# efirdc/Segmentation-Pipeline

Hardware: AMD Instinct MI355X
Metric: 3D patches/sec (128³, 4ch) train+infer at 1/2/4/8 MI355X; Dice vs CPU ref (higher is better)
Workload: dtype f32 (tensors, results and accumulation; the products of the 3x3x3 convolutions with >= 8 input channels run as six bf16 MFMAs on an EXACT three-way bf16 split of both f32 operands -- error vs f64 equal to the f32 MFMA kernels', profiles/r04_f32x3_accuracy.txt; the same step on v_mfma_f32_32x32x2_f32

## Files before the change

### segmentation-pipeline_amd/csrc/conv3d_f32x3.hip

```cpp
#include "conv3d_common.hpp"

namespace m355 {

typedef __bf16 bf16x8 __attribute__((ext_vector_type(8)));
typedef unsigned u32x4 __attribute__((ext_vector_type(4)));

constexpr int X3_PAIRS = 14;
constexpr int X3_QUADS = 7;
__host__ __device__ constexpr int x3_pair_tap(int pair, int half) {
  return pair < 9 ? pair * 3 + half : (pair < 12 ? (pair - 9) * 9 + half * 3 + 2 : (pair == 12 ? half * 9 + 8 : (half ? -1 : 26)));
}

__device__ __forceinline__ void x3_split(float v, unsigned& hi, unsigned& mid, unsigned& lo) {
  const unsigned u = __float_as_uint(v);
  hi = u & 0xffff0000u;
  const float r1 = (u & 0x7f800000u) == 0x7f800000u ? 0.f : v - __uint_as_float(hi);
  mid = __float_as_uint(r1) & 0xffff0000u;
  lo = __float_as_uint(r1 - __uint_as_float(mid));
}
__device__ __forceinline__ unsigned x3_pack(unsigned a, unsigned b) { return __builtin_amdgcn_perm(b, a, 0x07060302u); }

__device__ __forceinline__ void pack_w3_x3_item(const float* __restrict__ w, u32x4* __restrict__ wq, int64_t i, int Cout_w,
                                                int Cin_w, int kin, int mout, int nchunks, int transpose) {
  const int lane = (int)(i & 63);
// ... 987 lines not shown
  const dim3 grid((unsigned)(p.ctiles * p.otiles * p.nsplit));
#define M355_X3_BWW(TXV)                                                                                              \
  hipLaunchKernelGGL((conv3_bww_x3_kernel<TXV>), grid, dim3(512), 0, st, x, dy, slab, N, Cin, Cout, D, H, W, p.ty_tiles, \
                     p.tx_tiles, p.nsplit, p.ctiles, p.otiles, xbs, ybs);
  if (p.tx == 32) { M355_X3_BWW(32) } else if (p.tx == 16) { M355_X3_BWW(16) } else { M355_X3_BWW(8) }
#undef M355_X3_BWW
  return M355_OK;
}

template <int NVT>
__global__ __launch_bounds__(256) void convt_k2s2_fwd_x3_kernel(
    const float* __restrict__ x, const float* __restrict__ w, const float* __restrict__ bias, float* __restrict__ y, int Cin,
    int Cout, int D, int H, int W, int64_t xbs, int64_t ybs, int mt_per_wg) {
  extern __shared__ __attribute__((aligned(16))) unsigned char xs3_raw[];
  u32x4* xs3 = reinterpret_cast<u32x4*>(xs3_raw);
  constexpr int NG = NVT / 32, P = 256 / NVT;
  const int tid = threadIdx.x, lane = tid & 63;
  const int wave = __builtin_amdgcn_readfirstlane(tid >> 6);
  const int half = lane >> 5, l32 = lane & 31;
  const int S = D * H * W;
  const int v0 = blockIdx.x * NVT;
  const int n = blockIdx.z;
  const float* xn = x + (int64_t)n * xbs;
  float* yn = y + (int64_t)n * ybs;
  const int CB = (Cin + 15) / 16 * 2;
  const int OH = 2 * H, OW = 2 * W;
  const int64_t OS = (int64_t)S * 8;
  {
    const int sv = tid % NVT, part = tid / NVT;
    const bool vin = v0 + sv < S;
    const float* xp = xn + (vin ? v0 + sv : 0);
    for (int cb = part; cb < CB; cb += P) {
      float v[8];
#pragma unroll
      for (int j = 0; j < 8; ++j) {
        const int c = cb * 8 + j;
        const bool ok = vin && c < Cin;
        const float t = xp[ok ? (int64_t)c * S : 0];
        v[j] = ok ? t : 0.f;
      }
      unsigned h[8], m[8], l[8];
#pragma unroll
      for (int j = 0; j < 8; ++j) x3_split(v[j], h[j], m[j], l[j]);
      xs3[(0 * CB + cb) * NVT + sv] = (u32x4){x3_pack(h[0], h[1]), x3_pack(h[2], h[3]), x3_pack(h[4], h[5]), x3_pack(h[6], h[7])};
      xs3[(1 * CB + cb) * NVT + sv] = (u32x4){x3_pack(m[0], m[1]), x3_pack(m[2], m[3]), x3_pack(m[4], m[5]), x3_pack(m[6], m[7])};
      xs3[(2 * CB + cb) * NVT + sv] = (u32x4){x3_pack(l[0], l[1]), x3_pack(l[2], l[3]), x3_pack(l[4], l[5]), x3_pack(l[6], l[7])};
    }
  }
  __syncthreads();
  const int mtiles = (Cout + 3) / 4;
  const int mt_begin = blockIdx.y * mt_per_wg, mt_end = min(mtiles, mt_begin + mt_per_wg);
  const int wrow = Cout * 8;
  int64_t obase[NG];
#pragma unroll
  for (int g = 0; g < NG; ++g) {
    const int v = min(v0 + g * 32 + l32, S - 1);
    const int ix = v % W, iy = (v / W) % H, iz = v / (W * H);
    obase[g] = ((int64_t)(2 * iz + half) * OH + 2 * iy) * OW + 2 * ix;
  }
  float a_nxt[8];
  auto wload = [&](int mt, int k0) __attribute__((always_inline)) {
    const int col = min(mt * 32 + l32, Cout * 8 - 1);
#pragma unroll
    for (int j = 0; j < 8; ++j) a_nxt[j] = w[min(k0 + 8 * half + j, Cin - 1) * wrow + col];
  };
  bf16x8 ah, am, al;
  auto wsplit = [&](int mt, int k0) __attribute__((always_inline)) {
    const bool ook = mt * 4 + (l32 >> 3) < Cout;
    unsigned h[8], m[8], l[8];
#pragma unroll
    for (int j = 0; j < 8; ++j) x3_split((ook && k0 + 8 * half + j < Cin) ? a_nxt[j] : 0.f, h[j], m[j], l[j]);
    ah = __builtin_bit_cast(bf16x8, (u32x4){x3_pack(h[0], h[1]), x3_pack(h[2], h[3]), x3_pack(h[4], h[5]), x3_pack(h[6], h[7])});
    am = __builtin_bit_cast(bf16x8, (u32x4){x3_pack(m[0], m[1]), x3_pack(m[2], m[3]), x3_pack(m[4], m[5]), x3_pack(m[6], m[7])});
    al = __builtin_bit_cast(bf16x8, (u32x4){x3_pack(l[0], l[1]), x3_pack(l[2], l[3]), x3_pack(l[4], l[5]), x3_pack(l[6], l[7])});
  };
  const int nchunks = CB / 2;
  int mt = mt_begin + wave;
  if (mt < mt_end) {
    wload(mt, 0);
    wsplit(mt, 0);
  }
  while (mt < mt_end) {
    const int o0 = mt * 4;
    f32x16 acc[NG];
#pragma unroll
    for (int g = 0; g < NG; ++g)
#pragma unroll
      for (int r = 0; r < 16; ++r) acc[g][r] = 0.f;
    for (int ch = 0; ch < nchunks; ++ch) {
      const bool last = ch + 1 >= nchunks;
      const int nmt = last ? mt + 4 : mt, nk0 = last ? 0 : (ch + 1) * 16;
      if (nmt < mt_end) wload(nmt, nk0);
      const u32x4* bp = xs3 + (2 * ch + half) * NVT + l32;
      bf16x8 bh[NG], bm[NG], bl[NG];
#pragma unroll
      for (int g = 0; g < NG; ++g) bh[g] = __builtin_bit_cast(bf16x8, bp[g * 32]);
#pragma unroll
      for (int g = 0; g < NG; ++g) bm[g] = __builtin_bit_cast(bf16x8, bp[CB * NVT + g * 32]);
#pragma unroll
      for (int g = 0; g < NG; ++g) bl[g] = __builtin_bit_cast(bf16x8, bp[2 * CB * NVT + g * 32]);
#pragma unroll
      for (int g = 0; g < NG; ++g) acc[g] = __builtin_amdgcn_mfma_f32_32x32x16_bf16(al, bh[g], acc[g], 0, 0, 0);
#pragma unroll
      for (int g = 0; g < NG; ++g) acc[g] = __builtin_amdgcn_mfma_f32_32x32x16_bf16(am, bh[g], acc[g], 0, 0, 0);
#pragma unroll
      for (int g = 0; g < NG; ++g) acc[g] = __builtin_amdgcn_mfma_f32_32x32x16_bf16(ah, bh[g], acc[g], 0, 0, 0);
#pragma unroll
      for (int g = 0; g < NG; ++g) acc[g] = __builtin_amdgcn_mfma_f32_32x32x16_bf16(am, bm[g], acc[g], 0, 0, 0);
#pragma unroll
      for (int g = 0; g < NG; ++g) acc[g] = __builtin_amdgcn_mfma_f32_32x32x16_bf16(ah, bm[g], acc[g], 0, 0, 0);
#pragma unroll
      for (int g = 0; g < NG; ++g) acc[g] = __builtin_amdgcn_mfma_f32_32x32x16_bf16(ah, bl[g], acc[g], 0, 0, 0);
      wsplit(nmt, nk0);
    }
#pragma unroll
    for (int q = 0; q < 4; ++q) {
      const int o = o0 + q;
      if (o >= Cout) continue;
      const float bv = bias ? bias[o] : 0.f;
      float* yo = yn + (int64_t)o * OS;
#pragma unroll
      for (int g = 0; g < NG; ++g) {
        if (v0 + g * 32 + l32 >= S) continue;
#pragma unroll
        for (int b = 0; b < 2; ++b)
          *reinterpret_cast<float2*>(yo + obase[g] + (int64_t)b * OW) =
              make_float2(acc[g][q * 4 + b * 2] + bv, acc[g][q * 4 + b * 2 + 1] + bv);
      }
    }
    mt += 4;
  }
}

int convt_fwd_x3_nvt(int Cin) {
  const int64_t cin2 = round_up(Cin, 16);
  for (int nvt : {128, 64, 32})
    if (cin2 * nvt * 6 <= 65536) return nvt;
  return 0;
}

void launch_convt_fwd_x3(int nvt, dim3 grid, const float* x, const float* w, const float* bias, float* y, int Cin, int Cout,
                         int D, int H, int W, int64_t xbs, int64_t ybs, int mt_per_wg, hipStream_t st) {
  const size_t lds = (size_t)round_up(Cin, 16) * nvt * 6;
#define M355_CONVT_X3(NVT) \
  hipLaunchKernelGGL(convt_k2s2_fwd_x3_kernel<NVT>, grid, dim3(256), lds, st, x, w, bias, y, Cin, Cout, D, H, W, xbs, ybs, mt_per_wg)
  switch (nvt) {
    case 128: M355_CONVT_X3(128); break;
    case 64: M355_CONVT_X3(64); break;
    default: M355_CONVT_X3(32); break;
  }
#undef M355_CONVT_X3
}

}
```

### segmentation-pipeline_amd/csrc/convt.hip

```cpp
#include "h16.hpp"

namespace m355 {

typedef float f32x16 __attribute__((ext_vector_type(16)));

int convt_fwd_x3_nvt(int Cin);
void launch_convt_fwd_x3(int nvt, dim3 grid, const float* x, const float* w, const float* bias, float* y, int Cin, int Cout,
                         int D, int H, int W, int64_t xbs, int64_t ybs, int mt_per_wg, hipStream_t st);


template <int NVT>
__global__ __launch_bounds__(256) void convt_k2s2_fwd_mfma_kernel(
    const float* __restrict__ x, const float* __restrict__ w, const float* __restrict__ bias,
    float* __restrict__ y, int Cin, int Cout, int D, int H, int W, int64_t xbs, int64_t ybs, int mt_per_wg) {
  extern __shared__ float xs[];
  constexpr int NG = NVT / 32, P = 256 / NVT;
  const int tid = threadIdx.x, lane = tid & 63;
  const int wave = __builtin_amdgcn_readfirstlane(tid >> 6);
  const int half = lane >> 5, l32 = lane & 31;
  const int S = D * H * W;
  const int v0 = blockIdx.x * NVT;
  const int n = blockIdx.z;
  const float* xn = x + (int64_t)n * xbs;
  float* yn = y + (int64_t)n * ybs;
  constexpr int KC = 8;
  const int Cin2 = (Cin + 2 * KC - 1) / (2 * KC) * (2 * KC);
  const int OH = 2 * H, OW = 2 * W;
  const int64_t OS = (int64_t)S * 8;
  {
    const int sv = tid % NVT, part = tid / NVT;
    const bool vin = v0 + sv < S;
    const float* xp = xn + (vin ? v0 + sv : 0);
#pragma unroll 16
    for (int c = part; c < Cin2; c += P) {
      const bool ok = vin && c < Cin;
      const float val = xp[ok ? (int64_t)c * S : 0];
      xs[c * NVT + sv] = ok ? val : 0.f;
    }
  }
  __syncthreads();
  const int mtiles = (Cout + 3) / 4;
  const int mt_begin = blockIdx.y * mt_per_wg, mt_end = min(mtiles, mt_begin + mt_per_wg);
  const int wrow = Cout * 8;
  int64_t obase[NG];
#pragma unroll
  for (int g = 0; g < NG; ++g) {
    const int v = min(v0 + g * 32 + l32, S - 1);
    const int ix = v % W, iy = (v / W) % H, iz = v / (W * H);
    obase[g] = ((int64_t)(2 * iz + half) * OH + 2 * iy) * OW + 2 * ix;
  }
  float a_cur[KC], a_nxt[KC];
  auto wload = [&](float* a, int mt, int k0) {
    const int col = min(mt * 32 + l32, Cout * 8 - 1);
#pragma unroll
    for (int j = 0; j < KC; ++j) a[j] = w[min(k0 + 2 * j + half, Cin - 1) * wrow + col];
  };
  auto wmask = [&](float* dst, const float* src, int mt, int k0) {
    const bool ook = mt * 4 + (l32 >> 3) < Cout;
#pragma unroll
    for (int j = 0; j < KC; ++j) dst[j] = (ook && k0 + 2 * j + half < Cin) ? src[j] : 0.f;
  };
  const float* xb = xs + half * NVT + l32;
  int mt = mt_begin + wave;
  if (mt < mt_end) {
    wload(a_nxt, mt, 0);
    wmask(a_cur, a_nxt, mt, 0);
  }
  while (mt < mt_end) {
    const int o0 = mt * 4;
    f32x16 acc[NG];
#pragma unroll
    for (int g = 0; g < NG; ++g)
#pragma unroll
      for (int r = 0; r < 16; ++r) acc[g][r] = 0.f;
    for (int k0 = 0; k0 < Cin2; k0 += 2 * KC) {
      const bool last = k0 + 2 * KC >= Cin2;
      const int nmt = last ? mt + 4 : mt, nk0 = last ? 0 : k0 + 2 * KC;
      if (nmt < mt_end) wload(a_nxt, nmt, nk0);
      float bq[2][NG];
#pragma unroll
      for (int g = 0; g < NG; ++g) bq[0][g] = xb[k0 * NVT + g * 32];
#pragma unroll
      for (int j = 0; j < KC; ++j) {
        if (j + 1 < KC) {
#pragma unroll
          for (int g = 0; g < NG; ++g) bq[(j + 1) & 1][g] = xb[(k0 + 2 * j + 2) * NVT + g * 32];
        }
        __builtin_amdgcn_sched_barrier(0);
#pragma unroll
        for (int g = 0; g < NG; ++g)
          acc[g] = __builtin_amdgcn_mfma_f32_32x32x2f32(a_cur[j], bq[j & 1][g], acc[g], 0, 0, 0);
        __builtin_amdgcn_sched_barrier(0);
      }
      wmask(a_cur, a_nxt, nmt, nk0);
    }
#pragma unroll
    for (int q = 0; q < 4; ++q) {
      const int o = o0 + q;
      if (o >= Cout) continue;
      const float bv = bias ? bias[o] : 0.f;
      float* yo = yn + (int64_t)o * OS;
#pragma unroll
      for (int g = 0; g < NG; ++g) {
        if (v0 + g * 32 + l32 >= S) continue;
#pragma unroll
        for (int b = 0; b < 2; ++b)
          *reinterpret_cast<float2*>(yo + obase[g] + (int64_t)b * OW) =
              make_float2(acc[g][q * 4 + b * 2] + bv, acc[g][q * 4 + b * 2 + 1] + bv);
      }
    }
    mt += 4;
  }
}

template <int NVT, typename HT>
__global__ __launch_bounds__(256) void convt_k2s2_fwd_c8_kernel(
    const HT* __restrict__ x16, const float* __restrict__ w, const float* __restrict__ bias, HT* __restrict__ y16,
    int Cin, int Cout, int D, int H, int W, int64_t xbs16, int64_t ybs16, int mp_per_wg) {
  using hx8 = typename H16<HT>::x8;
  extern __shared__ float xs[];
  constexpr int NG = NVT / 32, P = 256 / NVT;
  const int tid = threadIdx.x, lane = tid & 63;
  const int wave = __builtin_amdgcn_readfirstlane(tid >> 6);
  const int half = lane >> 5, l32 = lane & 31;
  const int S = D * H * W;
  const int v0 = blockIdx.x * NVT;
  const int n = blockIdx.z;
  constexpr int KC = 8;
  const int Cin2 = (Cin + 2 * KC - 1) / (2 * KC) * (2 * KC);
  const int CBin = (Cin + 7) / 8;
  const int OH = 2 * H, OW = 2 * W;
  const int64_t OS = (int64_t)S * 8;
  {
    const int sv = tid % NVT, part = tid / NVT;
    const bool vin = v0 + sv < S;
    const hx8* xp = reinterpret_cast<const hx8*>(x16 + (int64_t)n * xbs16) + (vin ? v0 + sv : 0);
    for (int cb = part; cb < Cin2 / 8; cb += P) {
      const bool ok = vin && cb < CBin;
      const hx8 v = xp[ok ? (int64_t)cb * S : 0];
#pragma unroll
      for (int j = 0; j < 8; ++j) xs[(cb * 8 + j) * NVT + sv] = (ok && cb * 8 + j < Cin) ? (float)v[j] : 0.f;
    }
  }
  __syncthreads();
  const int mtiles = (Cout + 3) / 4, mpairs = (mtiles + 1) / 2;
  const int mp_begin = blockIdx.y * mp_per_wg, mp_end = min(mpairs, mp_begin + mp_per_wg);
  const int wrow = Cout * 8;
  int64_t obase[NG];
#pragma unroll
  for (int g = 0; g < NG; ++g) {
    const int v = min(v0 + g * 32 + l32, S - 1);
    const int ix = v % W, iy = (v / W) % H, iz = v / (W * H);
    obase[g] = ((int64_t)(2 * iz + half) * OH + 2 * iy) * OW + 2 * ix;
  }
  float a_cur[2][KC], a_nxt[2][KC];
  auto wload = [&](int mp, int k0) {
#pragma unroll
    for (int t = 0; t < 2; ++t) {
      const int col = min((2 * mp + t) * 32 + l32, Cout * 8 - 1);
#pragma unroll
      for (int j = 0; j < KC; ++j) a_nxt[t][j] = w[min(k0 + 2 * j + half, Cin - 1) * wrow + col];
// ... 748 lines not shown
  }
}

__global__ void convt_direct_bwd_data_kernel(const float* __restrict__ dy,
                                             const float* __restrict__ w, float* __restrict__ dx,
                                             int N, int Cin, int Cout, int D, int H, int W, int OD,
                                             int OH, int OW, int k, int stride, int pad,
                                             int64_t xbs, int64_t ybs) {
  const int64_t S = (int64_t)D * H * W;
  const int64_t OS = (int64_t)OD * OH * OW;
  const int64_t total = (int64_t)N * Cin * S;
  const int k3 = k * k * k;
  for (int64_t i = blockIdx.x * (int64_t)blockDim.x + threadIdx.x; i < total;
       i += (int64_t)gridDim.x * blockDim.x) {
    const int ix = (int)(i % W);
    int64_t r = i / W;
    const int iy = (int)(r % H);
    r /= H;
    const int iz = (int)(r % D);
    r /= D;
    const int c = (int)(r % Cin);
    const int n = (int)(r / Cin);
    float acc = 0.f;
    for (int o = 0; o < Cout; ++o) {
      const float* dyo = dy + (int64_t)n * ybs + (int64_t)o * OS;
      const float* wc = w + ((int64_t)c * Cout + o) * k3;
      for (int dz = 0; dz < k; ++dz) {
        const int oz = iz * stride + dz - pad;
        if (oz < 0 || oz >= OD) continue;
        for (int dyy = 0; dyy < k; ++dyy) {
          const int oy = iy * stride + dyy - pad;
          if (oy < 0 || oy >= OH) continue;
          for (int dxx = 0; dxx < k; ++dxx) {
            const int ox = ix * stride + dxx - pad;
            if (ox < 0 || ox >= OW) continue;
            acc = fmaf(dyo[((int64_t)oz * OH + oy) * OW + ox], wc[(dz * k + dyy) * k + dxx], acc);
          }
        }
      }
    }
    dx[(int64_t)n * xbs + (int64_t)c * S + ((int64_t)iz * H + iy) * W + ix] = acc;
  }
}

__global__ __launch_bounds__(256) void convt_direct_bwd_weight_kernel(
    const float* __restrict__ x, const float* __restrict__ dy, float* __restrict__ dw, int N, int Cin,
    int Cout, int D, int H, int W, int OD, int OH, int OW, int k, int stride, int pad, int64_t xbs,
    int64_t ybs) {
  __shared__ double scratch[4];
  const int k3 = k * k * k;
  int b = blockIdx.x;
  const int tap = b % k3;
  b /= k3;
  const int o = b % Cout;
  const int c = b / Cout;
  const int dz = tap / (k * k), dyy = (tap / k) % k, dxx = tap % k;
  const int64_t S = (int64_t)D * H * W;
  const int64_t OS = (int64_t)OD * OH * OW;
  double acc = 0.0;
  for (int n = 0; n < N; ++n) {
    const float* xc = x + (int64_t)n * xbs + (int64_t)c * S;
    const float* dyo = dy + (int64_t)n * ybs + (int64_t)o * OS;
    float part = 0.f;
    int cnt = 0;
    for (int64_t s = threadIdx.x; s < S; s += 256) {
      const int ix = (int)(s % W);
      const int iy = (int)((s / W) % H);
      const int iz = (int)(s / ((int64_t)W * H));
      const int oz = iz * stride + dz - pad, oy = iy * stride + dyy - pad,
                ox = ix * stride + dxx - pad;
      if (oz >= 0 && oz < OD && oy >= 0 && oy < OH && ox >= 0 && ox < OW)
        part = fmaf(xc[s], dyo[((int64_t)oz * OH + oy) * OW + ox], part);
      if (++cnt == 64) { acc += part; part = 0.f; cnt = 0; }
    }
    acc += part;
  }
  const double tot = block_sum<double, 256>(acc, scratch);
  if (threadIdx.x == 0) dw[((int64_t)c * Cout + o) * k3 + tap] = (float)tot;
}

static bool is_k2s2(const m355_conv3d_desc* d) {
  return d->k == 2 && d->stride == 2 && d->pad == 0 && d->out_pad == 0;
}
static int convt_out(int in, const m355_conv3d_desc* d) {
  return (in - 1) * d->stride - 2 * d->pad + d->k + d->out_pad;
}
static int convt_bww_mt(const m355_conv3d_desc* d) { return d->Cin > 64 ? 4 : 2; }
static int convt_nsplit(const m355_conv3d_desc* d) {
  const int64_t tiles = ceil_div(d->Cin, 32 * convt_bww_mt(d)) * ceil_div(d->Cout, 16);
  const int64_t nsteps = ceil_div((int64_t)d->N * d->D * d->H * d->W, 64);
  int64_t ns = std::max<int64_t>(1, 2 * num_cus() / tiles);
  ns = std::min<int64_t>(ns, nsteps);
  return (int)ns;
}
static bool convt_fits_i32(const m355_conv3d_desc* d) {
  return (int64_t)d->D * d->H * d->W * 8 * std::max(d->Cin, d->Cout) < (1ll << 31);
}

static int validate_convt(const m355_conv3d_desc* d, const char* who) {
  M355_REQUIRE(d != nullptr, M355_EINVALID_ARG, "%s: null descriptor", who);
  M355_REQUIRE(d->N > 0 && d->Cin > 0 && d->Cout > 0 && d->D > 0 && d->H > 0 && d->W > 0,
               M355_EINVALID_ARG, "%s: non-positive dimension", who);
  M355_REQUIRE(d->k >= 1 && d->k <= 7 && d->stride >= 1 && d->pad >= 0 && d->out_pad >= 0 &&
                   d->out_pad < d->stride,
               M355_EINVALID_ARG, "%s: bad k/stride/pad/out_pad", who);
  M355_REQUIRE(d->N <= 65535 && d->Cin <= 65535 && d->Cout <= 65535, M355_EUNSUPPORTED,
               "%s: N/Cin/Cout > 65535", who);
  return M355_OK;
}

}

using namespace m355;

int launch_dbias(const float* dy, float* dbias, int N, int Cout, int64_t S, int64_t ybs, void* ws,
                 hipStream_t st);
static size_t convt_slab_bytes(const m355_conv3d_desc* d) {
  return is_k2s2(d) ? (size_t)round_up((int64_t)convt_nsplit(d) * d->Cin * d->Cout * 8 * 4, 256) : 0;
}
static size_t convt_dbias_bytes(const m355_conv3d_desc* d) {
  const int64_t OS = (int64_t)convt_out(d->D, d) * convt_out(d->H, d) * convt_out(d->W, d);
  const int64_t generic = (int64_t)d->Cout * ceil_div(OS, DBIAS_CHUNK) * 8;
  const int64_t fused = is_k2s2(d) ? (int64_t)convt_nsplit(d) * d->Cout * 8 : 0;
  return (size_t)round_up(std::max(generic, fused), 256);
}

static int convt_fwd_nvt(const m355_conv3d_desc* d) {
  const int64_t cin2 = round_up(d->Cin, 16);
  for (int nvt : {128, 64, 32})
    if (cin2 * nvt * 4 <= 65536) return nvt;
  return 0;
}

struct ConvtBwdPlan {
  int mt, nvt, ksplit, o_per_split;
  size_t slab_bytes;
};
static ConvtBwdPlan plan_convt_bwd(const m355_conv3d_desc* d) {
  ConvtBwdPlan p{};
  const int64_t S = (int64_t)d->D * d->H * d->W;
  p.mt = d->Cin > 64 ? 4 : 2;
  const int64_t cblocks = ceil_div(d->Cin, 32 * p.mt);
  p.nvt = 256;
  while (p.nvt > 64 && ceil_div(S, p.nvt) * cblocks * d->N < 512) p.nvt >>= 1;
  const int64_t wgs = ceil_div(S, p.nvt) * cblocks * d->N;
  int64_t ks = 1;
  if (wgs < 256) ks = std::min<int64_t>(std::min<int64_t>(8, ceil_div(512, wgs)), std::max(1, d->Cout / 16));
  p.o_per_split = (int)round_up(ceil_div(d->Cout, ks), 4);
  p.ksplit = (int)ceil_div(d->Cout, p.o_per_split);
  p.slab_bytes = p.ksplit > 1 ? (size_t)round_up((int64_t)p.ksplit * d->N * d->Cin * S * 4, 256) : 0;
  return p;
}

extern "C" size_t m355_conv_transpose3d_workspace(const m355_conv3d_desc* d) {
  if (!d) return 0;
  const size_t bwd = is_k2s2(d) ? plan_convt_bwd(d).slab_bytes : 0;
  return std::max(convt_slab_bytes(d) + convt_dbias_bytes(d), bwd);
}

extern "C" int m355_conv_transpose3d_fwd(const m355_conv3d_desc* d, const float* x, const float* w,
                                         const float* bias, float* y, void* workspace,
                                         size_t workspace_bytes, void* stream) {
  if (int rc = validate_convt(d, "conv_transpose3d_fwd")) return rc;
  M355_REQUIRE(x && w && y, M355_EINVALID_ARG, "conv_transpose3d_fwd: null pointer");
  (void)workspace; (void)workspace_bytes;
  hipStream_t st = (hipStream_t)stream;
  const int OD = convt_out(d->D, d), OH = convt_out(d->H, d), OW = convt_out(d->W, d);
  M355_REQUIRE(OD > 0 && OH > 0 && OW > 0, M355_EINVALID_ARG, "conv_transpose3d_fwd: empty output");
  const int64_t xbs = dense_or(d->x_batch_stride, (int64_t)d->Cin * d->D * d->H * d->W);
  const int64_t ybs = dense_or(d->y_batch_stride, (int64_t)d->Cout * OD * OH * OW);
  const bool x3 = d->compute == M355_COMPUTE_F32X3 && tuning().f32x3 && tuning().f32x3_convt && convt_fwd_x3_nvt(d->Cin) != 0;
  const int nvt = x3 ? convt_fwd_x3_nvt(d->Cin) : convt_fwd_nvt(d);
  if (is_k2s2(d) && nvt && (ybs % 2 == 0) && ((uintptr_t)y & 7) == 0 && convt_fits_i32(d)) {
    const int64_t S = (int64_t)d->D * d->H * d->W;
    const int64_t vox_tiles = ceil_div(S, nvt) * d->N;
    const int mtiles = (int)ceil_div(d->Cout, 4);
    const int64_t groups = std::max<int64_t>(1, std::min<int64_t>(ceil_div(768, vox_tiles), ceil_div(mtiles, 4)));
    const int mt_per_wg = (int)round_up(ceil_div(mtiles, groups), 4);
    dim3 grid((unsigned)ceil_div(S, nvt), (unsigned)ceil_div(mtiles, mt_per_wg), (unsigned)d->N);
    if (x3) {
      launch_convt_fwd_x3(nvt, grid, x, w, bias, y, d->Cin, d->Cout, d->D, d->H, d->W, xbs, ybs, mt_per_wg, st);
      return check_launch("convt_k2s2_fwd_x3");
    }
    const size_t lds = (size_t)round_up(d->Cin, 16) * nvt * 4;
#define M355_CONVT_FWD(NVT)                                                                                   \
  hipLaunchKernelGGL(convt_k2s2_fwd_mfma_kernel<NVT>, grid, dim3(256), lds, st, x, w, bias, y, d->Cin, d->Cout, \
                     d->D, d->H, d->W, xbs, ybs, mt_per_wg)
    switch (nvt) {
      case 128: M355_CONVT_FWD(128); break;
      case 64: M355_CONVT_FWD(64); break;
      default: M355_CONVT_FWD(32); break;
    }
#undef M355_CONVT_FWD
    return check_launch("convt_k2s2_fwd");
  }
  const int64_t total = (int64_t)d->N * d->Cout * OD * OH * OW;
  const int blocks = (int)std::min<int64_t>(ceil_div(total, 256), 65535);
  hipLaunchKernelGGL(convt_direct_fwd_kernel, dim3(blocks), dim3(256), 0, st, x, w, bias, y, d->N,
                     d->Cin, d->Cout, d->D, d->H, d->W, OD, OH, OW, d->k, d->stride, d->pad, xbs, ybs);
  return check_launch("convt_direct_fwd");
}

extern "C" int m355_conv_transpose3d_fwd_h16(const m355_conv3d_desc* d, const void* x16, int64_t x16_batch_stride,
                                             const float* w, const float* bias, void* y16, int64_t y16_batch_stride,
                                             int32_t compute, void* stream) {
  if (int rc = validate_convt(d, "conv_transpose3d_fwd_h16")) return rc;
  M355_REQUIRE(x16 && w && y16, M355_EINVALID_ARG, "conv_transpose3d_fwd_h16: null pointer");
  M355_REQUIRE(compute == M355_COMPUTE_BF16 || compute == M355_COMPUTE_F16, M355_EINVALID_ARG,
               "conv_transpose3d_fwd_h16: compute must be M355_COMPUTE_BF16 or M355_COMPUTE_F16");
  const int nvt = std::min(convt_fwd_nvt(d), 64);
  M355_REQUIRE(is_k2s2(d) && nvt && convt_fits_i32(d), M355_EUNSUPPORTED,
               "conv_transpose3d_fwd_h16: only kernel_size 2 / stride 2 / padding 0 has a c8 kernel");
  const int64_t S = (int64_t)d->D * d->H * d->W;
  const int64_t xbs = dense_or(x16_batch_stride, c8_blocks(d->Cin) * S * 8);
  const int64_t ybs = dense_or(y16_batch_stride, c8_blocks(d->Cout) * S * 8 * 8);
  M355_REQUIRE((((uintptr_t)x16 | (uintptr_t)y16) & 15) == 0 && xbs % 8 == 0 && ybs % 8 == 0, M355_EINVALID_ARG,
               "conv_transpose3d_fwd_h16: c8 tensor not 16B aligned");
  hipStream_t st = (hipStream_t)stream;
  {
    const int ks_n = (int)ceil_div(d->Cin, 16);
    const int mtiles = 2 * (int)c8_blocks(d->Cout);
    if (S >= 16384 && ks_n <= 8 && tuning().convt_h16) {
      const int mt_per_wg = std::max(1, std::min(mtiles, 64 / ks_n));
      const int groups = (int)ceil_div(mtiles, mt_per_wg);
      const int ng = (S / 256) * groups * d->N >= 512 ? 2 : 1;
      const int64_t vox_tiles = ceil_div(S, 128 * ng);
      const int gx = (int)std::max<int64_t>(1, std::min<int64_t>(vox_tiles, ceil_div(512, (int64_t)groups * d->N)));
      dim3 grid((unsigned)gx, (unsigned)groups, (unsigned)d->N);
      const size_t lds = (size_t)mt_per_wg * ks_n * 1024;
#define M355_CONVT_H16(HT, KS, NG)                                                                                  \
  hipLaunchKernelGGL((convt_k2s2_fwd_h16_kernel<HT, KS, NG>), grid, dim3(256), lds, st, (const HT*)x16, w, bias,     \
                     (HT*)y16, d->Cin, d->Cout, d->D, d->H, d->W, xbs, ybs, mt_per_wg)
#define M355_CONVT_H16_T(HT)                                                         \
  if (ks_n <= 4) { if (ng == 2) M355_CONVT_H16(HT, 4, 2); else M355_CONVT_H16(HT, 4, 1); } \
  else { if (ng == 2) M355_CONVT_H16(HT, 8, 2); else M355_CONVT_H16(HT, 8, 1); }
      if (compute == M355_COMPUTE_BF16) { M355_CONVT_H16_T(__bf16) } else { M355_CONVT_H16_T(_Float16) }
#undef M355_CONVT_H16_T
#undef M355_CONVT_H16
      return check_launch("convt_k2s2_fwd_h16");
    }
  }
  const int64_t vox_tiles = ceil_div(S, nvt) * d->N;
  const int mpairs = (int)ceil_div(ceil_div(d->Cout, 4), 2);
  const int64_t groups = std::max<int64_t>(1, std::min<int64_t>(ceil_div(768, vox_tiles), ceil_div(mpairs, 4)));
  const int mp_per_wg = (int)round_up(ceil_div(mpairs, groups), 4);
  dim3 grid((unsigned)ceil_div(S, nvt), (unsigned)ceil_div(mpairs, mp_per_wg), (unsigned)d->N);
  const size_t lds = (size_t)round_up(d->Cin, 16) * nvt * 4;
#define M355_CONVT_C8(NVT, HT)                                                                                       \
  hipLaunchKernelGGL((convt_k2s2_fwd_c8_kernel<NVT, HT>), grid, dim3(256), lds, st, (const HT*)x16, w, bias, (HT*)y16, \
                     d->Cin, d->Cout, d->D, d->H, d->W, xbs, ybs, mp_per_wg)
  if (compute == M355_COMPUTE_BF16) {
    if (nvt == 64) M355_CONVT_C8(64, __bf16); else M355_CONVT_C8(32, __bf16);
  } else {
    if (nvt == 64) M355_CONVT_C8(64, _Float16); else M355_CONVT_C8(32, _Float16);
  }
#undef M355_CONVT_C8
  return check_launch("convt_k2s2_fwd_c8");
}

extern "C" int m355_conv_transpose3d_bwd_data(const m355_conv3d_desc* d, const float* dy,
                                              const float* w, float* dx, void* workspace,
                                              size_t workspace_bytes, void* stream) {
  if (int rc = validate_convt(d, "conv_transpose3d_bwd_data")) return rc;
  M355_REQUIRE(dy && w && dx, M355_EINVALID_ARG, "conv_transpose3d_bwd_data: null pointer");
  hipStream_t st = (hipStream_t)stream;
  const int OD = convt_out(d->D, d), OH = convt_out(d->H, d), OW = convt_out(d->W, d);
  const int64_t xbs = dense_or(d->x_batch_stride, (int64_t)d->Cin * d->D * d->H * d->W);
  const int64_t ybs = dense_or(d->y_batch_stride, (int64_t)d->Cout * OD * OH * OW);
  if (is_k2s2(d) && (ybs % 2 == 0) && ((uintptr_t)dy & 7) == 0 && convt_fits_i32(d)) {
    const int64_t S = (int64_t)d->D * d->H * d->W;
    const ConvtBwdPlan bp = plan_convt_bwd(d);
    const int mt = bp.mt, nvt = bp.nvt, ksplit = bp.ksplit;
    float* slab = nullptr;
    if (ksplit > 1) {
      M355_REQUIRE(workspace && workspace_bytes >= bp.slab_bytes, M355_EWORKSPACE,
                   "conv_transpose3d_bwd_data: workspace too small (%zu < %zu)", workspace_bytes, bp.slab_bytes);
      slab = (float*)workspace;
    }
    dim3 grid((unsigned)ceil_div(S, nvt), (unsigned)ceil_div(d->Cin, 32 * mt), (unsigned)(d->N * ksplit));
#define M355_CONVT_BWD(NVT, MT)                                                                                \
  hipLaunchKernelGGL((convt_k2s2_bwd_data_mfma_kernel<NVT, MT>), grid, dim3(256), 0, st, dy, w, dx, d->Cin,    \
                     d->Cout, d->D, d->H, d->W, xbs, ybs, ksplit, bp.o_per_split, slab)
    if (mt == 2) {
      if (nvt == 256) M355_CONVT_BWD(256, 2); else if (nvt == 128) M355_CONVT_BWD(128, 2); else M355_CONVT_BWD(64, 2);
    } else {
      if (nvt == 256) M355_CONVT_BWD(256, 4); else if (nvt == 128) M355_CONVT_BWD(128, 4); else M355_CONVT_BWD(64, 4);
    }
#undef M355_CONVT_BWD
    if (ksplit > 1) {
      const int64_t total = (int64_t)d->N * d->Cin * S;
      hipLaunchKernelGGL(convt_dx_reduce_kernel, dim3((unsigned)std::min<int64_t>(ceil_div(total, 256), 2048)), dim3(256),
                         0, st, slab, dx, d->N, (int64_t)d->Cin * S, xbs, ksplit);
    }
    return check_launch("convt_k2s2_bwd_data");
  }
  const int64_t total = (int64_t)d->N * d->Cin * d->D * d->H * d->W;
  const int blocks = (int)std::min<int64_t>(ceil_div(total, 256), 65535);
  hipLaunchKernelGGL(convt_direct_bwd_data_kernel, dim3(blocks), dim3(256), 0, st, dy, w, dx, d->N,
                     d->Cin, d->Cout, d->D, d->H, d->W, OD, OH, OW, d->k, d->stride, d->pad, xbs, ybs);
  return check_launch("convt_direct_bwd_data");
}

extern "C" int m355_conv_transpose3d_bwd_weight(const m355_conv3d_desc* d, const float* x,
                                                const float* dy, float* dw, float* dbias,
                                                void* workspace, size_t workspace_bytes,
                                                void* stream) {
  if (int rc = validate_convt(d, "conv_transpose3d_bwd_weight")) return rc;
  M355_REQUIRE(x && dy && dw, M355_EINVALID_ARG, "conv_transpose3d_bwd_weight: null pointer");
  hipStream_t st = (hipStream_t)stream;
  const int OD = convt_out(d->D, d), OH = convt_out(d->H, d), OW = convt_out(d->W, d);
  const int64_t xbs = dense_or(d->x_batch_stride, (int64_t)d->Cin * d->D * d->H * d->W);
  const int64_t ybs = dense_or(d->y_batch_stride, (int64_t)d->Cout * OD * OH * OW);
  if (is_k2s2(d) && (ybs % 2 == 0) && ((uintptr_t)dy & 7) == 0 && convt_fits_i32(d)) {
    const int nsplit = convt_nsplit(d);
    const size_t need = convt_slab_bytes(d);
    M355_REQUIRE(workspace && workspace_bytes >= need, M355_EWORKSPACE,
                 "conv_transpose3d_bwd_weight: workspace too small (%zu < %zu)", workspace_bytes,
                 need);
    float* slab = (float*)workspace;
    double* bslab = nullptr;
    if (dbias) {
      M355_REQUIRE(workspace_bytes >= need + convt_dbias_bytes(d), M355_EWORKSPACE,
                   "conv_transpose3d_bwd_weight: workspace too small for the bias gradient");
      bslab = (double*)((char*)workspace + need);
    }
    const int mt = convt_bww_mt(d);
    dim3 grid((unsigned)nsplit, (unsigned)ceil_div(d->Cout, 16), (unsigned)ceil_div(d->Cin, 32 * mt));
    if (mt == 2)
      hipLaunchKernelGGL(convt_k2s2_bwd_weight_mfma_kernel<2>, grid, dim3(256), 0, st, x, dy, slab, bslab, d->N,
                         d->Cin, d->Cout, d->D, d->H, d->W, xbs, ybs, nsplit);
    else
      hipLaunchKernelGGL(convt_k2s2_bwd_weight_mfma_kernel<4>, grid, dim3(256), 0, st, x, dy, slab, bslab, d->N,
                         d->Cin, d->Cout, d->D, d->H, d->W, xbs, ybs, nsplit);
    const int64_t total = (int64_t)d->Cin * d->Cout * 8;
    hipLaunchKernelGGL(convt_slab_reduce_kernel, dim3((unsigned)std::min<int64_t>(ceil_div(total, 256), 1024)),
                       dim3(256), 0, st, slab, dw, total, nsplit, bslab, dbias, d->Cout);
    return check_launch("conv_transpose3d_bwd_weight");
  } else {
    const int k3 = d->k * d->k * d->k;
    const int64_t nblk = (int64_t)d->Cin * d->Cout * k3;
    M355_REQUIRE(nblk < (1ll << 31), M355_EUNSUPPORTED, "conv_transpose3d_bwd_weight: grid too large");
    hipLaunchKernelGGL(convt_direct_bwd_weight_kernel, dim3((unsigned)nblk), dim3(256), 0, st, x, dy,
                       dw, d->N, d->Cin, d->Cout, d->D, d->H, d->W, OD, OH, OW, d->k, d->stride,
                       d->pad, xbs, ybs);
  }
  if (dbias) {
    M355_REQUIRE(workspace && workspace_bytes >= convt_slab_bytes(d) + convt_dbias_bytes(d), M355_EWORKSPACE,
                 "conv_transpose3d_bwd_weight: workspace too small for the bias gradient");
    launch_dbias(dy, dbias, d->N, d->Cout, (int64_t)OD * OH * OW, ybs, (char*)workspace + convt_slab_bytes(d), st);
  }
  return check_launch("conv_transpose3d_bwd_weight");
}

static bool convt_c8_bwd_ok(const m355_conv3d_desc* d) {
  const int64_t S = (int64_t)d->D * d->H * d->W;
  return is_k2s2(d) && 8 * ceil_div(c8_blocks(d->Cout), 2) <= 64 && S * 8 * 16 * 4 < (1ll << 31) &&
         S * 16 * std::min<int64_t>(16, c8_blocks(d->Cin)) < (1ll << 31);
}
static int convt_c8_ct(const m355_conv3d_desc* d) { const int ct = (int)ceil_div(d->Cin, 32); return ct >= 4 ? 4 : (ct >= 2 ? 2 : 1); }
static int convt_c8_nsplit(const m355_conv3d_desc* d) {
  const int64_t ntiles = (int64_t)d->N * d->D * ceil_div(d->H, 2) * ceil_div(d->W, 32);
  const int64_t groups = ceil_div(d->Cout, 32) * ceil_div(ceil_div(d->Cin, 32), convt_c8_ct(d));
  const int64_t wgs = (int64_t)(tuning().convt_wgs ? tuning().convt_wgs : 1) * num_cus();
  return (int)std::max<int64_t>(1, std::min<int64_t>(ntiles, wgs / groups));
}

extern "C" int32_t m355_conv_transpose3d_h16_bwd_supported(const m355_conv3d_desc* d) {
  return d && d->N > 0 && d->Cin > 0 && d->Cout > 0 && d->D > 0 && d->H > 0 && d->W > 0 && convt_c8_bwd_ok(d) ? 1 : 0;
}

extern "C" size_t m355_conv_transpose3d_h16_bwd_workspace(const m355_conv3d_desc* d) {
  if (!d || !m355_conv_transpose3d_h16_bwd_supported(d)) return 0;
  const int64_t OS = (int64_t)d->D * d->H * d->W * 8;
  return (size_t)round_up((int64_t)convt_c8_nsplit(d) * 8 * d->Cin * d->Cout * 4, 256) + dbias_c8_ws_bytes(d->N, d->Cout, OS);
}

extern "C" int m355_conv_transpose3d_bwd_data_h16(const m355_conv3d_desc* d, const void* dy16, int64_t dy16_batch_stride,
                                                  const float* w, void* dx16, int64_t dx16_batch_stride, int32_t compute,
                                                  void* stream) {
  if (int rc = validate_convt(d, "conv_transpose3d_bwd_data_h16")) return rc;
  M355_REQUIRE(dy16 && w && dx16, M355_EINVALID_ARG, "conv_transpose3d_bwd_data_h16: null pointer");
  M355_REQUIRE(compute == M355_COMPUTE_BF16 || compute == M355_COMPUTE_F16, M355_EINVALID_ARG,
               "conv_transpose3d_bwd_data_h16: compute must be M355_COMPUTE_BF16 or M355_COMPUTE_F16");
  M355_REQUIRE(convt_c8_bwd_ok(d), M355_EUNSUPPORTED,
               "conv_transpose3d_bwd_data_h16: only kernel_size 2 / stride 2 / padding 0 with Cout <= 128 has a c8 kernel "
               "(m355_conv_transpose3d_h16_bwd_supported)");
  const int64_t S = (int64_t)d->D * d->H * d->W;
  const int64_t ybs = dense_or(dy16_batch_stride, c8_blocks(d->Cout) * S * 8 * 8);
  const int64_t xbs = dense_or(dx16_batch_stride, c8_blocks(d->Cin) * S * 8);
  M355_REQUIRE((((uintptr_t)dy16 | (uintptr_t)dx16) & 15) == 0 && xbs % 8 == 0 && ybs % 8 == 0, M355_EINVALID_ARG,
               "conv_transpose3d_bwd_data_h16: c8 tensor not 16B aligned");
  hipStream_t st = (hipStream_t)stream;
  const int nks = 8 * (int)ceil_div(c8_blocks(d->Cout), 2);
  const int mtiles = (int)ceil_div(d->Cin, 32);
  int mt_per_wg = std::max(1, std::min(std::min(mtiles, 64 / nks), 4));
  if (mt_per_wg == 3) mt_per_wg = 2;
  const int groups = (int)ceil_div(mtiles, mt_per_wg);
  const int64_t vox_tiles = ceil_div(S, 128);
  const int64_t wgs = (int64_t)(tuning().convt_wgs ? tuning().convt_wgs : 2) * num_cus();
  const int gx = (int)std::max<int64_t>(1, std::min<int64_t>(ceil_div(vox_tiles, 4), ceil_div(wgs, (int64_t)groups * d->N)));
  dim3 grid((unsigned)gx, (unsigned)groups, (unsigned)d->N);
  const size_t lds = (size_t)mt_per_wg * nks * 1024;
#define M355_CTBD(HT, MTW)                                                                                            \
  hipLaunchKernelGGL((convt_k2s2_bwd_data_h16_kernel<HT, MTW>), grid, dim3(256), lds, st, (const HT*)dy16, w, (HT*)dx16, \
                     d->Cin, d->Cout, d->D, d->H, d->W, ybs, xbs, mt_per_wg,                                      \
                     compute == M355_COMPUTE_F16 ? overflow_flag() : nullptr)
#define M355_CTBD_T(HT)                                                  \
  if (mt_per_wg == 1) M355_CTBD(HT, 1); else if (mt_per_wg == 2) M355_CTBD(HT, 2); else M355_CTBD(HT, 4);
  if (compute == M355_COMPUTE_BF16) { M355_CTBD_T(__bf16) } else { M355_CTBD_T(_Float16) }
#undef M355_CTBD_T
#undef M355_CTBD
  return check_launch("convt_k2s2_bwd_data_h16");
}

extern "C" int m355_conv_transpose3d_bwd_weight_h16(const m355_conv3d_desc* d, const void* x16, int64_t x16_batch_stride,
                                                    const void* dy16, int64_t dy16_batch_stride, float* dw, float* dbias,
                                                    float grad_unscale, int32_t compute, void* workspace,
                                                    size_t workspace_bytes, void* stream) {
  if (int rc = validate_convt(d, "conv_transpose3d_bwd_weight_h16")) return rc;
  M355_REQUIRE(x16 && dy16 && dw && workspace, M355_EINVALID_ARG, "conv_transpose3d_bwd_weight_h16: null pointer");
  M355_REQUIRE(compute == M355_COMPUTE_BF16 || compute == M355_COMPUTE_F16, M355_EINVALID_ARG,
// ... 34 lines not shown
```

Before: 50.76.

## Add bf16x3-split MFMA kernel for transposed-conv backward-data

Adds a backward-data kernel for the k2s2 transposed convolution. It splits both f32 operands into three bf16 parts and accumulates six bf16 MFMAs, replacing the existing f32 MFMA path when f32x3 compute is selected. A new plan sizes per-wave tiles from the channel count and uses an output-channel k-split with a slab reduction to fill the SIMDs. This aims at higher matrix throughput, at the cost of extra split arithmetic, register pressure and a reduction pass.

```diff
diff --git a/segmentation-pipeline_amd/csrc/conv3d_f32x3.hip b/segmentation-pipeline_amd/csrc/conv3d_f32x3.hip
--- a/segmentation-pipeline_amd/csrc/conv3d_f32x3.hip
+++ b/segmentation-pipeline_amd/csrc/conv3d_f32x3.hip
@@ -1163,4 +1163,118 @@
 #undef M355_CONVT_X3
 }
 
-}
+template <int MTW, int NGW>
+__global__ __launch_bounds__(256) void convt_k2s2_bwd_data_x3_kernel(
+    const float* __restrict__ dy, const float* __restrict__ w, float* __restrict__ dx, int Cin, int Cout, int D, int H, int W,
+    int64_t xbs, int64_t ybs, int vblocks, int ksplit, int o_per_split, float* __restrict__ slab) {
+  const int tid = threadIdx.x, lane = tid & 63;
+  const int wave = __builtin_amdgcn_readfirstlane(tid >> 6);
+  const int half = lane >> 5, l32 = lane & 31;
+  const int vb = blockIdx.x * 4 + wave;
+  if (vb >= vblocks) return;
+  const int S = D * H * W;
+  const int c0 = blockIdx.y * MTW * 32;
+  const int n = (int)blockIdx.z / ksplit, ks = (int)blockIdx.z % ksplit;
+  const int o_lo = ks * o_per_split, o_hi = min(Cout, o_lo + o_per_split);
+  const float* dyn = dy + (int64_t)n * ybs;
+  const int OH = 2 * H, OW = 2 * W;
+  const int64_t OS = (int64_t)S * 8, OP = (int64_t)OH * OW;
+  const int vlane = vb * NGW * 32 + l32;
+  int64_t obase[NGW];
+#pragma unroll
+  for (int g = 0; g < NGW; ++g) {
+    const int v = min(vlane + g * 32, S - 1);
+    const int ix = v % W, iy = (v / W) % H, iz = v / (W * H);
+    obase[g] = ((int64_t)(2 * iz) * OH + 2 * iy) * OW + 2 * ix;
+  }
+  int64_t wrow[MTW];
+#pragma unroll
+  for (int m = 0; m < MTW; ++m) wrow[m] = (int64_t)min(c0 + m * 32 + l32, Cin - 1) * Cout * 8;
+
+  float braw[NGW][8], araw[MTW][8];
+  auto load = [&](int o0) __attribute__((always_inline)) {
+    const int oc = min(o0 + half, o_hi - 1);
+#pragma unroll
+    for (int g = 0; g < NGW; ++g) {
+      const float* p = dyn + oc * OS + obase[g];
+#pragma unroll
+      for (int ab = 0; ab < 4; ++ab) {
+        const float2 t = *reinterpret_cast<const float2*>(p + (ab >> 1) * OP + (ab & 1) * OW);
+        braw[g][2 * ab] = t.x;
+        braw[g][2 * ab + 1] = t.y;
+      }
+    }
+#pragma unroll
+    for (int m = 0; m < MTW; ++m) {
+      const float4* q = reinterpret_cast<const float4*>(w + wrow[m] + (int64_t)oc * 8);
+      const float4 a0 = q[0], a1 = q[1];
+      araw[m][0] = a0.x; araw[m][1] = a0.y; araw[m][2] = a0.z; araw[m][3] = a0.w;
+      araw[m][4] = a1.x; araw[m][5] = a1.y; araw[m][6] = a1.z; araw[m][7] = a1.w;
+    }
+  };
+  bf16x8 ah[MTW], am[MTW], al[MTW], bh[NGW], bm[NGW], bl[NGW];
+  auto split8 = [&](const float* r, bool ok, bf16x8& ph, bf16x8& pm, bf16x8& pl) __attribute__((always_inline)) {
+    unsigned h[8], m[8], l[8];
+#pragma unroll
+    for (int j = 0; j < 8; ++j) x3_split(ok ? r[j] : 0.f, h[j], m[j], l[j]);
+    ph = __builtin_bit_cast(bf16x8, (u32x4){x3_pack(h[0], h[1]), x3_pack(h[2], h[3]), x3_pack(h[4], h[5]), x3_pack(h[6], h[7])});
+    pm = __builtin_bit_cast(bf16x8, (u32x4){x3_pack(m[0], m[1]), x3_pack(m[2], m[3]), x3_pack(m[4], m[5]), x3_pack(m[6], m[7])});
+    pl = __builtin_bit_cast(bf16x8, (u32x4){x3_pack(l[0], l[1]), x3_pack(l[2], l[3]), x3_pack(l[4], l[5]), x3_pack(l[6], l[7])});
+  };
+
+  f32x16 acc[MTW][NGW];
+#pragma unroll
+  for (int m = 0; m < MTW; ++m)
+#pragma unroll
+    for (int g = 0; g < NGW; ++g)
+#pragma unroll
+      for (int r = 0; r < 16; ++r) acc[m][g][r] = 0.f;
+
+  load(o_lo);
+  for (int o0 = o_lo; o0 < o_hi; o0 += 2) {
+    const bool ok = o0 + half < o_hi;
+#pragma unroll
+    for (int g = 0; g < NGW; ++g) split8(braw[g], ok, bh[g], bm[g], bl[g]);
+#pragma unroll
+    for (int m = 0; m < MTW; ++m) split8(araw[m], ok, ah[m], am[m], al[m]);
+    if (o0 + 2 < o_hi) load(o0 + 2);
+#pragma unroll
+    for (int m = 0; m < MTW; ++m)
+#pragma unroll
+      for (int g = 0; g < NGW; ++g) {
+        acc[m][g] = __builtin_amdgcn_mfma_f32_32x32x16_bf16(al[m], bh[g], acc[m][g], 0, 0, 0);
+        acc[m][g] = __builtin_amdgcn_mfma_f32_32x32x16_bf16(am[m], bh[g], acc[m][g], 0, 0, 0);
+        acc[m][g] = __builtin_amdgcn_mfma_f32_32x32x16_bf16(ah[m], bh[g], acc[m][g], 0, 0, 0);
+        acc[m][g] = __builtin_amdgcn_mfma_f32_32x32x16_bf16(am[m], bm[g], acc[m][g], 0, 0, 0);
+        acc[m][g] = __builtin_amdgcn_mfma_f32_32x32x16_bf16(ah[m], bm[g], acc[m][g], 0, 0, 0);
+        acc[m][g] = __builtin_amdgcn_mfma_f32_32x32x16_bf16(ah[m], bl[g], acc[m][g], 0, 0, 0);
+      }
+  }
+  float* out = ksplit == 1 ? dx + (int64_t)n * xbs : slab + ((int64_t)ks * (gridDim.z / ksplit) + n) * Cin * S;
+#pragma unroll
+  for (int g = 0; g < NGW; ++g) {
+    const int v = vlane + g * 32;
+    if (v >= S) continue;
+#pragma unroll
+    for (int m = 0; m < MTW; ++m)
+#pragma unroll
+      for (int r = 0; r < 16; ++r) {
+        const int c = c0 + m * 32 + (r & 3) + 8 * (r >> 2) + 4 * half;
+        if (c < Cin) out[(int64_t)c * S + v] = acc[m][g][r];
+      }
+  }
+}
+
+void launch_convt_bwd_data_x3(int mtw, int ngw, dim3 grid, const float* dy, const float* w, float* dx, int Cin, int Cout, int D,
+                              int H, int W, int64_t xbs, int64_t ybs, int vblocks, int ksplit, int o_per_split, float* slab,
+                              hipStream_t st) {
+#define M355_CONVT_BWD_X3(MTW, NGW)                                                                                          \
+  hipLaunchKernelGGL((convt_k2s2_bwd_data_x3_kernel<MTW, NGW>), grid, dim3(256), 0, st, dy, w, dx, Cin, Cout, D, H, W, xbs, \
+                     ybs, vblocks, ksplit, o_per_split, slab)
+  if (mtw == 4) M355_CONVT_BWD_X3(4, 1);
+  else if (mtw == 2) M355_CONVT_BWD_X3(2, 2);
+  else M355_CONVT_BWD_X3(1, 2);
+#undef M355_CONVT_BWD_X3
+}
+
+}
diff --git a/segmentation-pipeline_amd/csrc/convt.hip b/segmentation-pipeline_amd/csrc/convt.hip
--- a/segmentation-pipeline_amd/csrc/convt.hip
+++ b/segmentation-pipeline_amd/csrc/convt.hip
@@ -7,6 +7,9 @@
 int convt_fwd_x3_nvt(int Cin);
 void launch_convt_fwd_x3(int nvt, dim3 grid, const float* x, const float* w, const float* bias, float* y, int Cin, int Cout,
                          int D, int H, int W, int64_t xbs, int64_t ybs, int mt_per_wg, hipStream_t st);
+void launch_convt_bwd_data_x3(int mtw, int ngw, dim3 grid, const float* dy, const float* w, float* dx, int Cin, int Cout, int D,
+                              int H, int W, int64_t xbs, int64_t ybs, int vblocks, int ksplit, int o_per_split, float* slab,
+                              hipStream_t st);
 
 
 template <int NVT>
@@ -1061,9 +1064,34 @@
   return p;
 }
 
+struct ConvtBwdX3Plan {
+  int mtw, ngw, mblocks, vblocks, ksplit, o_per_split;
+  size_t slab_bytes;
+};
+static bool convt_bwd_x3(const m355_conv3d_desc* d) {
+  return d->compute == M355_COMPUTE_F32X3 && tuning().f32x3 && tuning().f32x3_convt;
+}
+static ConvtBwdX3Plan plan_convt_bwd_x3(const m355_conv3d_desc* d) {
+  ConvtBwdX3Plan p{};
+  const int64_t S = (int64_t)d->D * d->H * d->W;
+  const int mtiles = (int)ceil_div(d->Cin, 32);
+  p.mtw = mtiles == 1 ? 1 : (mtiles % 4 == 0 ? 4 : 2);
+  p.ngw = p.mtw == 4 ? 1 : 2;
+  p.mblocks = (int)ceil_div(mtiles, p.mtw);
+  p.vblocks = (int)ceil_div(S, 32 * p.ngw);
+  const int64_t waves = (int64_t)p.mblocks * p.vblocks * d->N, simds = 4 * (int64_t)num_cus();
+  int64_t ks = 1;
+  if (waves < simds) ks = std::max<int64_t>(1, std::min<int64_t>({16, ceil_div(simds, waves), d->Cout / 8}));
+  p.o_per_split = (int)round_up(ceil_div(d->Cout, ks), 2);
+  p.ksplit = (int)ceil_div(d->Cout, p.o_per_split);
+  p.slab_bytes = p.ksplit > 1 ? (size_t)round_up((int64_t)p.ksplit * d->N * d->Cin * S * 4, 256) : 0;
+  return p;
+}
+
 extern "C" size_t m355_conv_transpose3d_workspace(const m355_conv3d_desc* d) {
   if (!d) return 0;
-  const size_t bwd = is_k2s2(d) ? plan_convt_bwd(d).slab_bytes : 0;
+  const size_t bwd = is_k2s2(d) ? std::max(plan_convt_bwd(d).slab_bytes, convt_bwd_x3(d) ? plan_convt_bwd_x3(d).slab_bytes : 0)
+                                : 0;
   return std::max(convt_slab_bytes(d) + convt_dbias_bytes(d), bwd);
 }
 
@@ -1176,6 +1204,26 @@
   const int OD = convt_out(d->D, d), OH = convt_out(d->H, d), OW = convt_out(d->W, d);
   const int64_t xbs = dense_or(d->x_batch_stride, (int64_t)d->Cin * d->D * d->H * d->W);
   const int64_t ybs = dense_or(d->y_batch_stride, (int64_t)d->Cout * OD * OH * OW);
+  if (is_k2s2(d) && (ybs % 2 == 0) && ((uintptr_t)dy & 7) == 0 && convt_fits_i32(d) && convt_bwd_x3(d) &&
+      ((uintptr_t)w & 15) == 0) {
+    const int64_t S = (int64_t)d->D * d->H * d->W;
+    const ConvtBwdX3Plan bp = plan_convt_bwd_x3(d);
+    float* slab = nullptr;
+    if (bp.ksplit > 1) {
+      M355_REQUIRE(workspace && workspace_bytes >= bp.slab_bytes, M355_EWORKSPACE,
+                   "conv_transpose3d_bwd_data: workspace too small (%zu < %zu)", workspace_bytes, bp.slab_bytes);
+      slab = (float*)workspace;
+    }
+    dim3 grid((unsigned)ceil_div(bp.vblocks, 4), (unsigned)bp.mblocks, (unsigned)(d->N * bp.ksplit));
+    launch_convt_bwd_data_x3(bp.mtw, bp.ngw, grid, dy, w, dx, d->Cin, d->Cout, d->D, d->H, d->W, xbs, ybs, bp.vblocks,
+                             bp.ksplit, bp.o_per_split, slab, st);
+    if (bp.ksplit > 1) {
+      const int64_t total = (int64_t)d->N * d->Cin * S;
+      hipLaunchKernelGGL(convt_dx_reduce_kernel, dim3((unsigned)std::min<int64_t>(ceil_div(total, 256), 2048)), dim3(256),
+                         0, st, slab, dx, d->N, (int64_t)d->Cin * S, xbs, bp.ksplit);
+    }
+    return check_launch("convt_k2s2_bwd_data_x3");
+  }
   if (is_k2s2(d) && (ybs % 2 == 0) && ((uintptr_t)dy & 7) == 0 && convt_fits_i32(d)) {
     const int64_t S = (int64_t)d->D * d->H * d->W;
     const ConvtBwdPlan bp = plan_convt_bwd(d);
```

After: 50.71, median of 6. About the same (-0.1%).
